# tobifinn/torch-assimilate

Hardware: AMD Instinct MI355X
Metric: local analyses/sec (LETKF, 40-member) (higher is better)
Workload: dtype f32

## Files before the change

### include/mia_letkf.h

```cpp
#ifndef MIA_LETKF_H
#define MIA_LETKF_H

#include <stddef.h>
#include <stdint.h>

#ifdef __cplusplus
extern "C" {
#endif

#define MIA_VERSION 100

#define MIA_OK 0
#define MIA_ERR_NULL (-1)
#define MIA_ERR_SIZE (-2)
#define MIA_ERR_UNSUPPORTED (-3)
#define MIA_ERR_WORKSPACE (-4)
#define MIA_ERR_ALIGN (-5)
#define MIA_ERR_COMM (-6)
#define MIA_ERR_ARG (-7)

#define MIA_FLAG_OVERFLOW 1
#define MIA_FLAG_NOCONV 2
#define MIA_FLAG_NONFINITE 4
#define MIA_FLAG_RETRY 8
#define MIA_FLAG_MASK 0xff

#define MIA_TAPER_GC 0
#define MIA_TAPER_GC_INF 1

#define MIA_MAX_COORD 3
#define MIA_MAX_RADII 3

int mia_version(void);
const char* mia_status_string(int status);

int mia_set_option(const char* name, int value);
int mia_get_option(const char* name, int* value);
int mia_last_analysis_kernel(char* buf, int n);
int mia_last_transform_kernel(char* buf, int n);

int mia_gaspari_cohn_f64(const double* r, int64_t n, double* w, void* stream);
int mia_gaspari_cohn_f32(const float* r, int64_t n, float* w, void* stream);
int mia_gaspari_cohn_inf_f64(const double* r, int64_t n, double* w, void* stream);
int mia_gaspari_cohn_inf_f32(const float* r, int64_t n, float* w, void* stream);

int mia_letkf_localize_workspace_bytes(int64_t P, int n_coord, size_t* bytes);
int mia_letkf_localize_f64(const double* grid_xyz, int64_t g0, int64_t g1,
                           const double* obs_xyz, int64_t P, int n_coord,
                           const int32_t* coord_group ,
                           const double* gc_c , int n_r, double gc_eps,
                           int p_cap, int32_t* nbr_cnt, int32_t* nbr_idx, double* nbr_w,
                           int32_t* stats, void* ws, size_t ws_bytes, void* stream);

int mia_letkf_localize_taper_f64(int taper, const double* grid_xyz, int64_t g0, int64_t g1,
                                 const double* obs_xyz, int64_t P, int n_coord,
                                 const int32_t* coord_group , const double* gc_c , int n_r,
                                 double gc_eps, int p_cap, int32_t* nbr_cnt, int32_t* nbr_idx, double* nbr_w,
                                 int32_t* stats, void* ws, size_t ws_bytes, void* stream);

int mia_letkf_index_build_f64(const double* obs_xyz, int64_t P, int n_coord,
                              const int32_t* coord_group , const double* gc_c , int n_r,
                              void* ws, size_t ws_bytes , void* stream);

int mia_letkf_localize_taper_periodic_f64(int taper, const double* grid_xyz, int64_t g0, int64_t g1,
                                          const double* obs_xyz, int64_t P, int n_coord,
                                          const int32_t* coord_group , const double* period ,
                                          const double* gc_c , int n_r, double gc_eps, int p_cap, int32_t* nbr_cnt, int32_t* nbr_idx, double* nbr_w,
                                          int32_t* stats, void* ws, size_t ws_bytes, void* stream);
int mia_letkf_index_build_periodic_f64(const double* obs_xyz, int64_t P, int n_coord,
                                       const int32_t* coord_group , const double* period ,
                                       const double* gc_c , int n_r, void* ws, size_t ws_bytes, void* stream);

// ... 427 lines not shown
```

### torch-assimilate_amd/_build.py

```python
import hashlib
import os
import shutil
import subprocess

HERE = os.path.dirname(os.path.abspath(__file__))
ROOT = os.path.dirname(HERE)
CSRC = os.path.join(HERE, "csrc")
LIB_DIR = os.path.join(HERE, "lib")
LIB_PATH = os.path.join(LIB_DIR, "libmia_letkf.so")
STAMP = os.path.join(LIB_DIR, "libmia_letkf.stamp")
SOURCES = ["localize.hip", "letkf_entry.hip", "etkf_global.hip", "letkf_wave.hip", "letkf_sys.hip", "letkf_cheb.hip", "letkf_tile.hip", "letkf_tile_split.hip", "letkf_tile64.hip", "letkf_tile64w.hip", "letkf_dense64.hip", "letkf_patch64.hip", "letkf_stream64.hip", "letkf_stream64w.hip", "letkf_patch64w.hip", "letkf_wide64.hip", "letkf_wide64w.hip", "letkf_tile2.hip", "letkf_tile2w.hip", "letkf_tile2p.hip", "letkf_tile2f.hip", "lketkf_tile.hip", "lketkf_tile64.hip", "lketkf_kern64.hip", "tile_lists.hip", "sharded_step.hip", "step_comm.hip", "obs_space.hip", "ienks.hip", "lienks_tile64.hip", "lienks_wide64.hip", "lienks_stream64.hip", "apply_local.hip", "apply_local64.hip", "api.cc"]
HEADERS = ["mia_common.h", "mia_options.h", "mia_jacobi.h", "mia_jacobi_sym.h", "mia_kernel_prog.h", "mia_localize_dev.h", "mia_kernels.h", "mia_cheb_table64.h", "mia_pack_dev.h", "mia_step_comm.h", "mia_tiles.h", "mia_tile_launch.h", "mia_frames64.h", os.path.join(ROOT, "include", "mia_letkf.h")]
INCLUDES = {"letkf_tile_split.hip": ["letkf_tile.hip"], "lketkf_kern64.hip": ["lketkf_tile64.hip"]}
SOURCE_FLAGS = {"letkf_tile2.hip": ["-fno-slp-vectorize"], "letkf_tile2w.hip": ["-fno-slp-vectorize"], "letkf_tile2p.hip": ["-fno-slp-vectorize"],
                "letkf_tile2f.hip": ["-fno-slp-vectorize"]}
FLAGS = ["--offload-arch=gfx950", "-O3", "-std=c++17", "-fPIC", "-shared",
         "-I" + os.path.join(ROOT, "include"), "-I" + CSRC]


def _flags():
    return FLAGS + os.environ.get("MIA_BUILD_FLAGS", "").split()


def _sources():
    return [os.path.join(CSRC, s) for s in SOURCES if os.path.exists(os.path.join(CSRC, s))]


def _digest():
    h = hashlib.sha256()
    for f in _sources() + [f if os.path.isabs(f) else os.path.join(CSRC, f) for f in HEADERS]:
        with open(f, "rb") as fh:
            h.update(fh.read())
    h.update(" ".join(_flags()).encode())
    return h.hexdigest()


def hipcc_path():
    return shutil.which("hipcc") or "/opt/rocm/bin/hipcc"


def _object_digest(src):
    h = hashlib.sha256()
    for f in [src] + [f if os.path.isabs(f) else os.path.join(CSRC, f) for f in HEADERS + INCLUDES.get(os.path.basename(src), [])]:
        with open(f, "rb") as fh:
            h.update(fh.read())
# ... 54 lines not shown
```

### torch-assimilate_amd/_cabi.py

```python
import ctypes as C
import os

from ._build import LIB_PATH

_lib = None

i32, i64, f32, f64, vp, sz = C.c_int, C.c_int64, C.c_float, C.c_double, C.c_void_p, C.c_size_t


class KernelOp(C.Structure):
    _fields_ = [("op", C.c_int32), ("reserved", C.c_int32), ("value", C.c_double)]


_LISTS = [vp, vp, vp, i32, i32]
_SHARD = [vp, i64, i32, i32, i64, i64, vp, i64] + _LISTS


def _analysis_entry(f):
    return (_SHARD + [f, f, vp, i64, i64, vp, vp, vp], i32)


def _analysis_redo(f):
    return (_SHARD + [f, f, vp, i64, i64, vp, vp], i32)


def _weights_entry(f):
    return (_SHARD + [f, f, vp, i64, i64, vp, vp, vp, vp], i32)


def _ienks_tile_entry(f):
    return ([vp, i64, i32, i64, i64, vp, i64] + _LISTS + [f, vp, vp, vp, vp], i32)


_COVER7 = ([i32, i32, i32, i64, i64, i64, i64], i32)
_COVER4 = ([i32, i32, i64, i64], i32)

_PROTOS = {
    "mia_version": ([], i32),
    "mia_status_string": ([i32], C.c_char_p),
    "mia_set_option": ([C.c_char_p, i32], i32),
    "mia_get_option": ([C.c_char_p, C.POINTER(C.c_int)], i32),
    "mia_last_analysis_kernel": ([C.c_char_p, i32], i32),
    "mia_last_transform_kernel": ([C.c_char_p, i32], i32),
    "mia_gaspari_cohn_f64": ([vp, i64, vp, vp], i32),
    "mia_gaspari_cohn_f32": ([vp, i64, vp, vp], i32),
    "mia_gaspari_cohn_inf_f64": ([vp, i64, vp, vp], i32),
    "mia_gaspari_cohn_inf_f32": ([vp, i64, vp, vp], i32),
    "mia_letkf_localize_taper_f64": ([i32, vp, i64, i64, vp, i64, i32, C.POINTER(C.c_int32), C.POINTER(f64), i32, f64,
                                      i32, vp, vp, vp, vp, vp, sz, vp], i32),
    "mia_letkf_localize_from_dist_taper_f64": ([i32, vp, vp, i64, i32, C.POINTER(f64), i32, f64, vp, vp, vp, vp, vp],
                                               i32),
    "mia_lketkf_kernel_analysis_packed_f32": ([vp, i64, i32, i32, i64, i64, vp, i64, vp, vp, vp, i32, i32, f32,
                                               C.POINTER(KernelOp), i32, vp, i64, i64, vp, vp, vp], i32),
    "mia_lketkf_kernel_analysis_packed_f64": ([vp, i64, i32, i32, i64, i64, vp, i64, vp, vp, vp, i32, i32, f64,
                                               C.POINTER(KernelOp), i32, vp, i64, i64, vp, vp, vp], i32),
    "mia_letkf_localize_workspace_bytes": ([i64, i32, C.POINTER(sz)], i32),
    "mia_letkf_localize_f64": ([vp, i64, i64, vp, i64, i32, C.POINTER(C.c_int32), C.POINTER(f64), i32, f64,
                                i32, vp, vp, vp, vp, vp, sz, vp], i32),
    "mia_letkf_localize_from_dist_f64": ([vp, vp, i64, i32, C.POINTER(f64), i32, f64, vp, vp, vp, vp, vp], i32),
    "mia_letkf_analysis_workspace_bytes": ([i32, i64, i32, C.POINTER(sz)], i32),
    "mia_letkf_analysis_f32": ([vp, i64, i32, i32, i64, i64, vp, vp, i64, vp, vp, vp, i32, i32, f32,
                                vp, i64, i64, vp, vp, vp, sz, vp], i32),
    "mia_letkf_analysis_f64": ([vp, i64, i32, i32, i64, i64, vp, vp, i64, vp, vp, vp, i32, i32, f64,
                                vp, i64, i64, vp, vp, vp, sz, vp], i32),
    "mia_letkf_pack_obs_f32": ([vp, vp, i32, i64, vp, vp], i32),
    "mia_letkf_pack_obs_f64": ([vp, vp, i32, i64, vp, vp], i32),
    "mia_letkf_analysis_packed_f32": _analysis_entry(f32),
    "mia_letkf_analysis_packed_f64": _analysis_entry(f64),
    "mia_letkf_analysis_matfun_f32": _analysis_entry(f32),
    "mia_letkf_analysis_matfun_f64": _analysis_entry(f64),
    "mia_letkf_analysis_retry_f64": _analysis_redo(f64),
    "mia_letkf_matfun_f64_cover": _COVER7,
    "mia_letkf_analysis_dense_f64": _analysis_entry(f64),
    "mia_letkf_dense_f64_cover": _COVER7,
    "mia_letkf_analysis_patch_f64": ([vp, i64, i32, i32, i64, i64, vp, i64, vp, vp, vp, i32, i32, f64, f64,
                                      vp, i64, i64, vp, vp, vp, i64, i32, vp], i32),
# ... 221 lines not shown
```

### torch-assimilate_amd/csrc/api.cc

```cpp
#include "mia_letkf.h"

extern "C" int mia_version(void) { return MIA_VERSION; }

extern "C" const char* mia_status_string(int status) {
  switch (status) {
    case MIA_OK: return "ok";
    case MIA_ERR_NULL: return "required pointer is NULL";
    case MIA_ERR_SIZE: return "invalid or inconsistent size argument";
    case MIA_ERR_UNSUPPORTED: return "shape not supported by the gfx950 kernels (LDS capacity / index range)";
    case MIA_ERR_WORKSPACE: return "workspace too small (use the *_workspace_bytes query)";
    case MIA_ERR_ALIGN: return "workspace pointer must be 256-byte aligned";
    case MIA_ERR_COMM: return "RCCL / communicator failure (mia_comm_last_error has the detail)";
    case MIA_ERR_ARG: return "invalid argument value (e.g. a negative or non-finite period)";
    default: return status > 0 ? "HIP runtime error (value is the hipError_t)" : "unknown status";
  }
}

#include <atomic>
#include <cstring>
#include "mia_options.h"

namespace mia {
static std::atomic<int> g_opt[MIA_OPT_COUNT_] = {62, 1, 1, 1, 1, 1, 1, 1, 1, 1, 1, 1, 1, 1};
static thread_local const int* t_override = nullptr;
int option(int id) {
  if (id < 0 || id >= MIA_OPT_COUNT_) return 0;
  return t_override ? t_override[id] : g_opt[id].load(std::memory_order_relaxed);
}
void option_snapshot(int* out) { for (int i = 0; i < MIA_OPT_COUNT_; ++i) out[i] = g_opt[i].load(std::memory_order_relaxed); }
void option_override(const int* snapshot) { t_override = snapshot; }
static std::atomic<int> g_apply64{-1};
int option_apply64() { return g_apply64.load(std::memory_order_relaxed); }
}

#include <cstdarg>
#include <cstdio>
#include <mutex>
namespace mia {
static std::mutex g_last_mu;
static char g_last_kernel[160] = "";
void note_analysis_kernel(const char* fmt, ...) {
  char buf[sizeof(g_last_kernel)];
  va_list ap;
  va_start(ap, fmt);
  vsnprintf(buf, sizeof(buf), fmt, ap);
  va_end(ap);
  std::lock_guard<std::mutex> lk(g_last_mu);
  memcpy(g_last_kernel, buf, sizeof(buf));
}
}

extern "C" int mia_last_analysis_kernel(char* buf, int n) {
  if (!buf || n < 1) return MIA_ERR_NULL;
  std::lock_guard<std::mutex> lk(mia::g_last_mu);
  snprintf(buf, (size_t)n, "%s", mia::g_last_kernel);
  return MIA_OK;
}

namespace mia {
static char g_last_transform[160] = "";
void note_transform_kernel(const char* fmt, ...) {
  char buf[sizeof(g_last_transform)];
  va_list ap;
  va_start(ap, fmt);
  vsnprintf(buf, sizeof(buf), fmt, ap);
  va_end(ap);
// ... 39 lines not shown
```

### torch-assimilate_amd/csrc/letkf_tile2.hip

```cpp
#include "mia_common.h"
#include <hip/hip_ext.h>
#include "mia_kernels.h"
#include "mia_options.h"
#include "mia_tiles.h"
#include "mia_tile_launch.h"
#include "letkf_tile2_kernel.h"

namespace mia {


template <int UT, int KT, bool MROWS, int WAVES>
__global__ __launch_bounds__(64, WAVES)
void letkf_tile2_kernel(Tile2Params P) { tile2_body<UT, KT, MROWS, 0>(P, nullptr, (int64_t)blockIdx.y * gridDim.x + blockIdx.x); }

#ifdef MIA_TILE_STAMPS
extern "C" int mia_debug_tile2_stamps(long long* host, int n_tiles) {
  if (n_tiles > kT2StampTiles) n_tiles = kT2StampTiles;
  return (int)hipMemcpyFromSymbol(host, HIP_SYMBOL(g_tile2_stamps), sizeof(long long) * kT2StampN * (size_t)n_tiles);
}
#endif

size_t tile2_lds_bytes(int ut, int k) {
  return (size_t)ut * split_nc8(k) * 512 + 512 + (size_t)16 * ut * 12;
}

template <int UT, int KT, bool MROWS>
constexpr int tile2_waves() { return UT <= 2 && KT <= 4 ? (MROWS ? 2 : MIA_TILE2_WAVES_UT2) : (UT <= 3 && KT <= 4 && !MROWS ? 2 : 1); }

template <int UT, int KT, bool MROWS, int WAVES = tile2_waves<UT, KT, MROWS>()>
static int tile2_launch_m(const Tile2Params& tp, hipStream_t stream) {
  size_t lds = tile2_lds_bytes(UT, tp.k);
  {
    int per_cu = 0;
    MIA_EXP_SET(per_cu, "MIA_TILE2_WAVES_PER_CU", atoi);
    if (per_cu > 0 && (size_t)(160 * 1024) / per_cu > lds) lds = ((size_t)(160 * 1024) / per_cu) & ~(size_t)255;
  }
  return launch_blocks_carried(letkf_tile2_kernel<UT, KT, MROWS, WAVES>, (tp.ng + 15) >> 4, 64, lds, stream, [] {
    note_analysis_kernel("letkf_tile2_kernel<%d, %d, %s, %d>", UT, KT, MROWS ? "true" : "false", WAVES);
  }, tp);
}

template <int UT, int KT>
static int tile2_launch_s(const Tile2Params& tp, hipStream_t stream) {
#ifdef MIA_EXPERIMENTS
  if constexpr (UT == 2 && KT == 3) {
    int w = 0;
    MIA_EXP_SET(w, "MIA_TILE2_WAVES", atoi);
    if (tp.m == 1 && w == 5) return tile2_launch_m<UT, KT, false, 5>(tp, stream);
    if (tp.m == 1 && w == 6) return tile2_launch_m<UT, KT, false, 6>(tp, stream);
    if (tp.m == 1 && w == 3) return tile2_launch_m<UT, KT, false, 3>(tp, stream);
  }
#endif
  bool force_rows = false;
  MIA_EXP_SET(force_rows, "MIA_TILE2_FORCE_MROWS", (bool)atoi);
  return tp.m == 1 && !force_rows ? tile2_launch_m<UT, KT, false>(tp, stream) : tile2_launch_m<UT, KT, true>(tp, stream);
}

template <int UT>
static int tile2_launch_u(const Tile2Params& tp, int kt, hipStream_t stream) {
  return dispatch_upto<6>(kt, [&](auto kt_c) {
    if constexpr (kt_c() >= 5 || UT <= kt_c() + 1) return tile2_launch_s<UT, kt_c()>(tp, stream);
    else return MIA_ERR_UNSUPPORTED;
  });
}

bool tile2_covers(int m, int k, int p_max, int extra_blocks, int64_t ldx, int64_t ldo, int64_t ng) {
  if (!(m >= 1 && k >= 2 && k <= 96 && p_max <= k && extra_blocks >= 0)) return false;
  if ((int64_t)k * ldx * 4 >= ((int64_t)1 << 31) || (int64_t)k * ldo * 4 >= ((int64_t)1 << 31)) return false;
  const int kt = (k + 15) >> 4, ut = tile_ut_for(p_max) + extra_blocks;
  if (ut > kt + 1 || ut > 6) return false;
  if (tile2_lds_bytes(ut, k) > kMaxDynamicLds) return false;
  return grid_covers((ng + 15) >> 4);
}

bool tile2_records_addressable(int k, int64_t P) { return (P + 1) * (int64_t)split_rec_bytes(k) < ((int64_t)1 << 32); }

int tile2_analysis_launch(const float* X, int64_t ldx, int m, int k, int64_t g0, int64_t ng, const void* rec, int64_t P,
                          const void* tile_lists, int ut, float inf_factor, float* Xa, int64_t ldo, int64_t o0,
                          int32_t* flags, int32_t* retry_count, int dmax, const int2* tab_hdr, const float2* tab_c,
                          hipStream_t stream, int seg_len, int64_t seg_stride, const Tile2Housekeeping* hk, const Tile2Loc* loc) {
  if (seg_len < 0 || (seg_len & 15) || (seg_len > 0 && ng >= ((int64_t)1 << 31))) return MIA_ERR_UNSUPPORTED;
  if (!flags || !retry_count || !tab_hdr || !tab_c || !tile_lists || !rec) return MIA_ERR_UNSUPPORTED;
  const int kt = (k + 15) >> 4;
  if (ut < 1 || ut > 6 || ut > kt + 1 || !tile2_covers(m, k, 0, ut - 1, ldx, ldo, ng)) return MIA_ERR_UNSUPPORTED;
  if (!tile2_records_addressable(k, P)) return MIA_ERR_UNSUPPORTED;
  const TileListLayout L = tile_list_layout(ng, ut);
  const char* base = (const char*)tile_lists;
  Tile2Params tp;
  tp.X = X; tp.ldx = ldx; tp.m = m; tp.k = k; tp.g0 = g0; tp.ng = ng;
  tp.rec = (const unsigned char*)rec; tp.rb = split_rec_bytes(k); tp.nc8 = split_nc8(k); tp.zero_rec = P;
  tp.thdr = (const int4*)(base + L.hdr); tp.tidx = (const int32_t*)(base + L.idx); tp.tD = (const f4w*)(base + L.D);
  const double rg = (double)(k - 1) / (double)inf_factor, km = (double)(k - 1);
  tp.inv_reg = (float)(1.0 / rg);
  tp.f0 = (float)sqrt(km / rg);
  tp.inv_k = (float)(1.0 / (double)k);
  tp.cs_phi = (float)(sqrt(km) / (rg * sqrt(rg)));
  tp.cs_psi = (float)(1.0 / rg);
  tp.Xa = Xa; tp.ldo = ldo; tp.o0 = o0; tp.flags = flags; tp.retry_count = retry_count; tp.dmax = dmax;
  tp.tab_hdr = tab_hdr; tp.tab_c = tab_c;
  tp.seg_len = seg_len; tp.seg_stride = seg_stride;
  tp.clr_counts = hk ? hk->counts : nullptr; tp.clr_n = hk ? hk->n : nullptr; tp.clr_err = hk ? hk->err : nullptr;
  tp.err_out = hk ? hk->err_out : nullptr;
  tp.stagger = 0;
  MIA_EXP_SET(tp.stagger, "MIA_TILE2_STAGGER", atoi);
  { int pm = 0, tr = 0; MIA_EXP_SET(pm, "MIA_TILE2_PRIO", atoi); MIA_EXP_SET(tr, "MIA_TILE2_TRIM", atoi); tp.stagger |= (pm & 0xff) << 8 | tr << 16; }
  if (loc) return tile2f_launch(tp, *loc, ut, kt, stream);
  if (ut >= 3 && option(MIA_OPT_TILE_PAIR) != 0) {
    const int prc = tile2p_launch_any(tp, ut, kt, stream);
    if (prc != MIA_ERR_UNSUPPORTED) return prc;
  }
#ifdef MIA_TILE2_SINGLE
  if (ut == 2 && kt == 3) return tile2_launch_s<2, 3>(tp, stream);
  return MIA_ERR_UNSUPPORTED;
#else
  return dispatch_upto<6>(ut, [&](auto ut_c) { return tile2_launch_u<ut_c()>(tp, kt, stream); });
#endif
}

}

using namespace mia;

extern "C" int mia_letkf_analysis_tiles_f32(const float* X, int64_t ldx, int m, int k, int64_t g0, int64_t g1,
                                            const void* split_rec, int64_t P, const void* tile_lists, int p_max,
                                            int extra_blocks, float inf_factor, float* Xa, int64_t ldo, int64_t o0, int32_t* flags,
                                            int32_t* retry_count, void* stream_) {
  (void)hipGetLastError();
  hipStream_t stream = (hipStream_t)stream_;
  if (m < 1 || k < 2 || g1 < g0 || g0 < 0 || P < 0 || p_max < 0 || extra_blocks < 0 || !(inf_factor > 0.0f)) return MIA_ERR_SIZE;
  if (g1 == g0) return MIA_OK;
  if (!X || !Xa || !split_rec || !tile_lists || !flags || !retry_count) return MIA_ERR_NULL;
  if (!tile2_covers(m, k, p_max, extra_blocks, ldx, ldo, g1 - g0)) return MIA_ERR_UNSUPPORTED;
  const int2* th = nullptr;
  const float2* tc = nullptr;
  if (!cheb_dual_table(stream, &th, &tc)) return MIA_ERR_UNSUPPORTED;
  return tile2_analysis_launch(X, ldx, m, k, g0, g1 - g0, split_rec, P, tile_lists, tile_ut_for(p_max) + extra_blocks, inf_factor, Xa,
// ... 3 lines not shown
```

### torch-assimilate_amd/csrc/letkf_tile2_kernel.h

```cpp
#pragma once
#include <type_traits>
#include "mia_common.h"
#include <hip/hip_ext.h>
#include "mia_kernels.h"
#include "mia_options.h"
#include "mia_tiles.h"
#ifdef MIA_TILE_STAMPS
namespace mia { constexpr int kT2StampN = 20, kT2StampTiles = 8192; static __device__ long long g_tile2_stamps[kT2StampTiles * kT2StampN]; }
#define MIA_TL_STAMP(i) do { if (lane == 0 && tile < mia::kT2StampTiles) mia::g_tile2_stamps[tile * mia::kT2StampN + 12 + (i)] = (long long)__builtin_amdgcn_s_memtime(); } while (0)
#endif
#include "mia_tile_localize.h"

namespace mia {

#ifdef MIA_TILE_STAMPS
#define T2_STAMP(i) do { if (lane == 0 && bid < kT2StampTiles) g_tile2_stamps[bid * kT2StampN + (i)] = (long long)__builtin_amdgcn_s_memtime(); } while (0)
#define T2_STAMP_HWID() do { if (lane == 0 && bid < kT2StampTiles) g_tile2_stamps[bid * kT2StampN + 9] = \
    (long long)(unsigned)__builtin_amdgcn_s_getreg((31 << 11) | 4) | ((long long)(unsigned)__builtin_amdgcn_s_getreg((31 << 11) | 20) << 32); } while (0)
#define T2_STAMP_REAL(i) do { if (lane == 0 && bid < kT2StampTiles) g_tile2_stamps[bid * kT2StampN + (i)] = (long long)__builtin_amdgcn_s_memrealtime(); } while (0)
#else
#define T2_STAMP(i) do { } while (0)
#define T2_STAMP_HWID() do { } while (0)
#define T2_STAMP_REAL(i) do { } while (0)
#endif

#ifndef MIA_TILE2_WAVES_UT2
#define MIA_TILE2_WAVES_UT2 4
#endif

template <int UT, int KT, bool MROWS, int LOC>
__device__ __forceinline__ void tile2_body(Tile2Params P, const Tile2Loc* loc, const int64_t bid) {
  constexpr int UMAX = 16 * UT, NB = (KT + 1) / 2, NKB = (UT + 1) / 2;
  extern __shared__ __attribute__((aligned(16))) unsigned char smem[];
  int lane = threadIdx.x, lr = lane & 15, h = lane >> 4;
  const int k = P.k, nc8 = P.nc8;
  const unsigned IMG = (unsigned)(UT * nc8) * 512u;
  unsigned char* zline = smem + IMG;
  int* ukey = reinterpret_cast<int*>(smem + IMG + 512);
  float* wdl = reinterpret_cast<float*>(ukey + UMAX);
  float* El = wdl + UMAX;

  const int64_t ntile = (P.ng + 15) >> 4;
  if (bid >= ntile) return;
  if (P.clr_counts) {
    const int ncl = *P.clr_n;
    for (int64_t i = bid * 64 + lane; i < ncl; i += ntile * 64) P.clr_counts[i] = 0;
    if (bid == 0 && lane == 0) {
      const unsigned e = *P.clr_err;
      if (e) { atomicOr(P.err_out, (int)(e << 3)); *P.clr_err = 0u; }
    }
  }
  const int64_t q8 = ntile >> 3, r8 = ntile & 7, xcd = bid & 7;
  const int64_t tile = (xcd < r8 ? xcd * (q8 + 1) : r8 * (q8 + 1) + (xcd - r8) * q8) + (bid >> 3);
  const int64_t p0 = tile << 4;
  const int npts = P.ng - p0 < 16 ? (int)(P.ng - p0) : 16;
  int64_t oc0 = P.o0 + p0;
  if (P.seg_len > 0) {
    const unsigned sgi = (unsigned)p0 / (unsigned)P.seg_len;
    oc0 = p0 - (int64_t)sgi * P.seg_len;
    P.Xa += (int64_t)sgi * P.seg_stride;
  }
  const unsigned ldxb = (unsigned)P.ldx * 4u, ldob = (unsigned)P.ldo * 4u;
  int lrc = lr < npts ? lr : npts - 1;
  bool colok = lr < npts;

#ifdef MIA_EXPERIMENTS
  const int prio_mode = (P.stagger >> 8) & 0xff, exp_trim = P.stagger >> 16;
  P.stagger &= 0xff;
  if (prio_mode == 1) __builtin_amdgcn_s_setprio(3);
  if (prio_mode >= 3) {
    const int wid = (int)(__builtin_amdgcn_s_getreg((4 << 11) | 4) & 0xf);
    const bool fast = prio_mode == 3 ? (wid & 1) : (prio_mode == 4 ? wid < 2 : (prio_mode == 5 ? wid == 0 : (wid % 3) == 0));
    if (fast) __builtin_amdgcn_s_setprio(3);
  }
  if (P.stagger > 0) {
    const int slot = (int)(__builtin_amdgcn_s_getreg((4 << 11) | 4) & 0xf);
    for (int i = 0; i < slot * P.stagger; ++i) __builtin_amdgcn_s_sleep(1);
  }
#endif
  T2_STAMP(0);
  T2_STAMP_HWID();
  T2_STAMP_REAL(10);
  int hdU = 0;
  int myidx[(UMAX + 63) / 64];
  f4w dreg[UT];
  if constexpr (LOC == 0) {
// ... 455 lines not shown
```

### torch-assimilate_amd/csrc/letkf_tile2f.hip

```cpp
#include "mia_common.h"
#include <hip/hip_ext.h>
#include "mia_kernels.h"
#include "mia_options.h"
#include "mia_tiles.h"
#include "mia_tile_launch.h"
#include "letkf_tile2_kernel.h"

namespace mia {

struct Tile2FParams { Tile2Params t; Tile2Loc loc; };

template <int UT, int KT, int NC, bool MROWS, int WAVES>
__global__ __launch_bounds__(64, WAVES)
void letkf_tile2f_kernel(Tile2FParams PF) { tile2_body<UT, KT, MROWS, NC>(PF.t, &PF.loc, (int64_t)blockIdx.y * gridDim.x + blockIdx.x); }

#ifdef MIA_TILE_STAMPS
extern "C" int mia_debug_tile2f_stamps(long long* host, int n_tiles) {
  if (n_tiles > kT2StampTiles) n_tiles = kT2StampTiles;
  return (int)hipMemcpyFromSymbol(host, HIP_SYMBOL(g_tile2_stamps), sizeof(long long) * kT2StampN * (size_t)n_tiles);
}
#endif

bool tile2f_covers(int m, int k, int ut, int n_coord) {
  const int kt = (k + 15) >> 4;
  return m >= 1 && ut >= 1 && ut <= 2 && kt >= 1 && kt <= 6 && n_coord >= 1 && n_coord <= MIA_MAX_COORD;
}

template <int UT, int KT, int NC, bool MROWS>
static int tile2f_launch_m(const Tile2FParams& pf, hipStream_t stream) {
  const size_t a = tile2_lds_bytes(UT, pf.t.k), b = tile_loc_lds(UT);
  const size_t lds = a > b ? a : b;
  constexpr int WAVES = MROWS ? 2 : MIA_TILE2_WAVES_UT2;
  return launch_blocks_carried(letkf_tile2f_kernel<UT, KT, NC, MROWS, WAVES>, (pf.t.ng + 15) >> 4, 64, lds, stream, [] {
    note_analysis_kernel("letkf_tile2f_kernel<%d, %d, %d, %s, %d>", UT, KT, NC, MROWS ? "true" : "false", WAVES);
  }, pf);
}

template <int UT, int KT, int NC>
static int tile2f_launch_n(const Tile2FParams& pf, hipStream_t stream) {
  return pf.t.m == 1 ? tile2f_launch_m<UT, KT, NC, false>(pf, stream) : tile2f_launch_m<UT, KT, NC, true>(pf, stream);
}

template <int UT>
static int tile2f_launch_u(const Tile2FParams& pf, int kt, hipStream_t stream) {
  return dispatch_upto<6>(kt, [&](auto kt_c) {
    return dispatch_among<7, 6, 5, 3, 2, 1>(pf.loc.scan.nc + (pf.loc.periodic ? 4 : 0), [&](auto nc) { return tile2f_launch_n<UT, kt_c(), nc()>(pf, stream); });
  });
}

int tile2f_launch(const Tile2Params& tp, const Tile2Loc& loc, int ut, int kt, hipStream_t stream) {
  if (!tile2f_covers(tp.m, tp.k, ut, loc.scan.nc) || !loc.stats) return MIA_ERR_UNSUPPORTED;
  Tile2FParams pf;
  pf.t = tp;
  pf.loc = loc;
#ifdef MIA_TILE2_SINGLE
  if (ut == 2 && kt == 3 && loc.scan.nc == 1) return tile2f_launch_n<2, 3, 1>(pf, stream);
  return MIA_ERR_UNSUPPORTED;
#else
  return ut == 1 ? tile2f_launch_u<1>(pf, kt, stream) : tile2f_launch_u<2>(pf, kt, stream);
#endif
}

}
```

### torch-assimilate_amd/csrc/mia_tile_launch.h

```cpp
#pragma once
#include <hip/hip_ext.h>
#include <type_traits>
#include <utility>
#include "mia_common.h"
#include "mia_kernels.h"

namespace mia {

constexpr int64_t kGridColumns = 65536, kGridMaxRows = 65535;
constexpr int64_t kGridMaxBlocks = kGridColumns * kGridMaxRows;
static inline bool grid_covers(int64_t n) { return n <= kGridMaxBlocks; }
static inline bool launch_grid(int64_t n, dim3* grid) {
  const int64_t gx = n < kGridColumns ? n : kGridColumns;
  const int64_t gy = (n + gx - 1) / gx;
  if (gy > kGridMaxRows) return false;
  *grid = dim3((unsigned)gx, (unsigned)gy);
  return true;
}

template <bool CARRIED, typename Note, typename... KArgs, typename... Args>
static inline int launch_blocks_impl(void (*kern)(KArgs...), int64_t n_blocks, unsigned block, size_t lds, hipStream_t stream, Note&& note,
                                     const Args&... args) {
  if (lds > kMaxDynamicLds) return MIA_ERR_UNSUPPORTED;
  if (lds > 48 * 1024) MIA_HIP_TRY(hipFuncSetAttribute((const void*)kern, hipFuncAttributeMaxDynamicSharedMemorySize, (int)lds));
  dim3 grid;
  if (!launch_grid(n_blocks, &grid)) return MIA_ERR_UNSUPPORTED;
  if constexpr (CARRIED) {
    hipEvent_t& stop = launch_stop_event();
    if (stop) {
      hipExtLaunchKernelGGL(kern, grid, dim3(block), (unsigned)lds, stream, launch_start_event(), stop, 0, args...);
      stop = nullptr;
      launch_start_event() = nullptr;
    } else {
      kern<<<grid, dim3(block), lds, stream>>>(args...);
    }
    ++tile_launch_count();
  } else {
    kern<<<grid, dim3(block), lds, stream>>>(args...);
  }
  note();
  MIA_LAUNCH_CHECK();
  return MIA_OK;
}
template <typename Note, typename... KArgs, typename... Args>
static inline int launch_blocks(void (*kern)(KArgs...), int64_t n_blocks, unsigned block, size_t lds, hipStream_t stream, Note&& note,
                                const Args&... args) {
  return launch_blocks_impl<false>(kern, n_blocks, block, lds, stream, note, args...);
}
template <typename Note, typename... KArgs, typename... Args>
static inline int launch_blocks_carried(void (*kern)(KArgs...), int64_t n_blocks, unsigned block, size_t lds, hipStream_t stream, Note&& note,
                                        const Args&... args) {
  return launch_blocks_impl<true>(kern, n_blocks, block, lds, stream, note, args...);
}
static inline void no_note() {}

template <int... Vs, typename F>
static inline int dispatch_among(int v, F&& f) {
  int rc = MIA_ERR_UNSUPPORTED;
  (void)((v == Vs ? (rc = f(std::integral_constant<int, Vs>{}), true) : false) || ...);
  return rc;
}
template <typename F, int... Is>
static inline int dispatch_upto_impl(int v, F&& f, std::integer_sequence<int, Is...>) { return dispatch_among<(int)(sizeof...(Is) - Is)...>(v, f); }
template <int N, typename F>
static inline int dispatch_upto(int v, F&& f) { return dispatch_upto_impl(v, f, std::make_integer_sequence<int, N>{}); }

}
```

### torch-assimilate_amd/csrc/mia_tiles.h

```cpp
#pragma once
#include "mia_common.h"

namespace mia {

constexpr int kTileSlack = 8;

static inline int tile_ut_for(int p_max) {
  const int ut = (p_max + kTileSlack + 15) >> 4;
  return ut < 1 ? 1 : ut;
}

struct TileListLayout { size_t hdr, idx, D, bytes; int ut; int64_t ntile; };
static inline TileListLayout tile_list_layout(int64_t ng, int ut) {
  TileListLayout L;
  L.ut = ut;
  L.ntile = (ng + 15) >> 4;
  size_t o = 0;
  L.hdr = o; o = align_up(o + (size_t)(L.ntile > 0 ? L.ntile : 1) * 16, 256);
  L.idx = o; o = align_up(o + (size_t)(L.ntile > 0 ? L.ntile : 1) * 16 * ut * sizeof(int32_t), 256);
  L.D = o; o = align_up(o + (size_t)(L.ntile > 0 ? L.ntile : 1) * ut * 1024, 256);
  L.bytes = o;
  return L;
}

// ... 285 lines not shown
  unsigned char* o = J.rec + j * rb;
  const float E = bad ? __builtin_nanf("") : __uint_as_float((unsigned)(127 - es) << 23);
  *reinterpret_cast<f4w*>(o + 32 * nc8) = f4w{wd, E, 0.0f, 0.0f};
  for (int c = 0; c < nc8; ++c) {
    float x[8];
#pragma unroll
    for (int i = 0; i < 8; ++i) x[i] = (real && 8 * c + i < k) ? lds[(8 * c + i) * 64 + lane] * sc : 0.0f;
    h8v hi, lo;
    split8(x, hi, lo);
    *reinterpret_cast<h8v*>(o + 32 * c) = hi;
    *reinterpret_cast<h8v*>(o + 32 * c + 16) = lo;
  }
}
static inline size_t split_pack_lean_lds(int k) { return (size_t)64 * k * sizeof(float); }

struct ScanParams;
int split_pack_launch(const float* Yb, const float* d, int k, int64_t P, void* rec, hipStream_t stream);
int tile_lists_launch(const double* grid_xyz, int64_t g0, int64_t ng, int64_t P, int n_coord, const int32_t* coord_group,
                      const double* gc_c, int n_r, double gc_eps, int taper, int ut, void* tile_lists, int32_t* stats,
                      void* index_ws, hipStream_t stream, const SplitPackJob* pack, bool bucket = false, const int* counts = nullptr,
                      const double* period = nullptr);
struct Tile2Params {
  const float* X; int64_t ldx; int m, k;
  int64_t g0, ng;
  const unsigned char* rec; int rb, nc8; int64_t zero_rec;
  const int4* thdr; const int32_t* tidx; const f4w* tD;
  float inv_reg, f0, inv_k, cs_phi, cs_psi;
  float* Xa; int64_t ldo, o0; int32_t* flags; int32_t* retry_count;
  int dmax;
  const int2* tab_hdr; const float2* tab_c;
  int seg_len; int64_t seg_stride;
  int* clr_counts; const int* clr_n; unsigned* clr_err; int32_t* err_out;
  int stagger;
};
struct Tile2Housekeeping { int* counts; const int* n; unsigned* err; int32_t* err_out; };
bool tile2_covers(int m, int k, int p_max, int extra_blocks, int64_t ldx, int64_t ldo, int64_t ng);
bool tile2_records_addressable(int k, int64_t P);
int tile2_analysis_launch(const float* X, int64_t ldx, int m, int k, int64_t g0, int64_t ng, const void* rec, int64_t P,
                          const void* tile_lists, int ut, float inf_factor, float* Xa, int64_t ldo, int64_t o0,
                          int32_t* flags, int32_t* retry_count, int dmax, const int2* tab_hdr, const float2* tab_c,
                          hipStream_t stream, int seg_len = 0, int64_t seg_stride = 0, const Tile2Housekeeping* hk = nullptr,
                          const struct Tile2Loc* loc = nullptr);
bool tile2f_covers(int m, int k, int ut, int n_coord);
int tile2f_launch(const Tile2Params& tp, const struct Tile2Loc& loc, int ut, int kt, hipStream_t stream);
size_t tile2_lds_bytes(int ut, int k);

int tile2p_launch_any(const Tile2Params& tp, int ut, int kt, hipStream_t stream);
bool lketkf_tile_covers(int m, int k, int p_max, int extra_blocks, int64_t ldx, int64_t ldo, int64_t ng, int64_t P);
int lketkf_tile_launch(const float* X, int64_t ldx, int m, int k, int64_t g0, int64_t ng, const float* Yb, const float* d,
                       int64_t P, const void* tile_lists, int ut, float inf_factor, float gamma, float* Xa, int64_t ldo,
                       int64_t o0, int32_t* flags, int32_t* retry_count, int dmax, const int2* tab_hdr, const float2* tab_c,
                       hipStream_t stream, int seg_len = 0, int64_t seg_stride = 0, const Tile2Housekeeping* hk = nullptr);

}
```

### torch-assimilate_amd/engine.py

```python
from __future__ import annotations

import ctypes as C
import warnings
from dataclasses import dataclass
from typing import Optional, Sequence

import torch

from . import _cabi

__all__ = ["LetkfEngine", "NeighbourLists", "ObsIndex", "mesh_tiles"]


def _ptr(t: Optional[torch.Tensor]):
    return None if t is None else C.c_void_p(t.data_ptr())


def _one_of(names) -> str:
    return ", ".join(repr(v) for v in names[:-1]) + " or " + repr(names[-1])


def _result(out, W, flags, finish, defer_retry):
    if not defer_retry:
        if finish is not None:
# ... 99 lines not shown

@dataclass
class ObsIndex:
    ws: torch.Tensor
    obs: torch.Tensor
    radii: list
    coord_group: list
    P: int
    nc: int
    period: Optional[list] = None


def _periods(period, nc: int):
    if period is None:
        return None
    per = [0.0 if p is None else float(p) for p in (period if hasattr(period, "__len__") else [period] * nc)]
    if len(per) != nc:
        raise ValueError("period needs one entry per coordinate")
    if any(not (p >= 0.0 and p < float("inf")) for p in per):
        raise ValueError("period must be finite and >= 0")
    if not any(p > 0.0 for p in per):
        return None
    return (C.c_double * nc)(*per)


def _period_arg(per, nc: int):
    return per if per is not None else (C.c_double * nc)()


class LetkfEngine:

    def __init__(self, device: Optional[torch.device] = None):
        self.lib = _cabi.lib()
        if not torch.cuda.is_available():
            raise _cabi.MiaError("no MI355X visible: the LETKF hot path has no CPU fallback")
        self.device = torch.device(device if device is not None else "cuda:%d" % torch.cuda.current_device())
        self._ws = {}
        self._p_cap_hint = 32

    def _stream(self):
        return C.c_void_p(torch.cuda.current_stream(self.device).cuda_stream)

    def _workspace(self, tag: str, nbytes: int) -> torch.Tensor:
        cur = self._ws.get(tag)
        if cur is None or cur.numel() < nbytes:
            cur = torch.empty(max(int(nbytes), 256), dtype=torch.uint8, device=self.device)
            assert cur.data_ptr() % 256 == 0
            self._ws[tag] = cur
        return cur

    def _dev(self, a, dtype):
        t = torch.as_tensor(a)
        return t.to(device=self.device, dtype=dtype).contiguous()

    def _redo_behind_counter(self, retry: torch.Tensor, entry: str, redo_args, alive=()):
        def finish(_alive=alive):
            n_retry = int(retry.item())
            if n_retry:
                _cabi.check(getattr(self.lib, entry)(*redo_args(), self._stream()), entry)
            return n_retry
        return finish

    def gaspari_cohn(self, r: torch.Tensor, taper: int = 0) -> torch.Tensor:
        r = r.to(self.device).contiguous()
        out = torch.empty_like(r)
        name = "mia_gaspari_cohn_" + ("inf_" if taper else "") + {torch.float64: "f64", torch.float32: "f32"}[r.dtype]
# ... 909 lines not shown
```

### torch-assimilate_amd/sharded.py

```python
from __future__ import annotations

from typing import Callable, List, Optional, Sequence, Tuple

import os
import torch

__all__ = ["ShardedLetkf", "PendingStep", "block_partition", "gather_blocks"]


TILE_BOX_OVERFLOW = 1 << 30
STATUS_NONFINITE = 128
STATUS_SAMPLED = 64


def block_partition(G: int, world: int) -> List[Tuple[int, int]]:
    n = (G + world - 1) // world
    return [(min(G, r * n), min(G, (r + 1) * n)) for r in range(world)]


def gather_blocks(shard: torch.Tensor, G: int, world: int, group=None) -> torch.Tensor:
    import torch.distributed as dist
    if world == 1:
        return shard
    m, k, n_r = shard.shape
# ... 137 lines not shown
        import ctypes as C
        from .engine import _ptr
        lib, comm = self.engine.lib, st["comm"]
        parts = block_partition(G, self.world)
        g0, g1 = parts[self.rank]
        col = torch.arange(G, device=self.device, dtype=torch.float32)
        ctr = torch.zeros(8, dtype=torch.int32, device=self.device)
        ok = True
        for s, buf in enumerate(bufs):
            flat = buf.view(rows, G)
            flat.fill_(-1.0)
            pat = lambda r, a, b: (r + 1) * 4096.0 + (col[a:b] % 61.0)[None] + (torch.arange(rows, device=self.device) % 64)[:, None] * 64.0
            flat[:, g0:g1] = pat(self.rank, g0, g1)
            torch.cuda.synchronize(self.device)
            ctr.zero_()
            ctr[0] = 100 + self.rank
            rc = lib.mia_comm_peer_exchange(comm, s, rows, G, g0, g1, _ptr(ctr), C.c_void_p(torch.cuda.current_stream(self.device).cuda_stream))
            torch.cuda.synchronize(self.device)
            want = torch.empty_like(flat)
            for r, (a, b) in enumerate(parts):
                want[:, a:b] = pat(r, a, b)
            c = ctr.tolist()
            ok = ok and rc == 0 and bool(torch.equal(flat, want)) and c[4] == 100 + self.world - 1 and c[7] == 0
        return ok

    def __init__(self, device, rank: int = 0, world: int = 1, radii: Sequence[float] = (10.0,),
                 inf_factor: float = 1.0, coord_group: Optional[Sequence[int]] = None, eps: float = 1e-5,
                 rbf_gamma: Optional[float] = None, compute_shard: Optional[Callable] = None, group=None,
                 method: str = "auto", fused_localization: bool = False,
                 comm_chunks: int = 4, chunk_compute: Optional[Callable] = None, native_step: bool = True,
                 max_in_flight: int = 3, peer_exchange: str = "auto", copy_results: bool = True, prep_streams: int = 3,
                 analysis_streams: int = 3, gather: bool = True, fuse_tile_lists="auto", prep_priority: int = 0, period=None):
        self.device, self.rank, self.world = device, rank, world
        self.radii, self.inf_factor, self.coord_group, self.eps = list(radii), inf_factor, coord_group, eps
        self.period = period
        self.rbf_gamma = rbf_gamma
        self.gather = bool(gather)
        self.method = method
        self.fused_localization = fused_localization
        self.fuse_tile_lists = fuse_tile_lists
        self.comm_chunks = int(comm_chunks)
        self._chunk_compute = chunk_compute
        self._comm_stream = None
        self._obuf = None
        self.native_step = native_step
        self._native = None
        self._in_flight = []
        self._time_next = False
        self.kernel_timings = []
        self.max_in_flight = max(1, min(int(max_in_flight), 16))
        self.prep_streams = max(0, min(int(prep_streams), 8))
        self.analysis_streams = max(1, min(int(analysis_streams), 4))
        self.prep_priority = int(prep_priority)
        self.peer_rewaits = 3
        self._peer_rewait_hook = None
        self.peer_exchange = peer_exchange
        self.copy_results = copy_results
        self._submitted = 0
        self.reused_steps = 0
        self._force_comm = False
        self.native_steps = 0
        self.last_retries = 0
        self.group = group
        self._engine = None
        self._compute = compute_shard or self._engine_shard
        self.last_p_max = 0
# ... 907 lines not shown
```

Before: 2.612 billion.

## Pack multiple tile wavefronts per workgroup in tile2 LETKF kernels

Tile2 kernels previously launched one 64-thread wavefront per block. Each workgroup now holds up to four wavefronts (default 4, set by MIA_TILE_WPG), each processing its own tile in a private LDS slice. The XCD-aware tile mapping now applies at group granularity. This cuts the block count and may improve scheduling and occupancy, but it raises launch bounds to 256 threads, which can constrain registers, and it couples four waves' LDS into one allocation.

```diff
diff --git a/include/mia_letkf.h b/include/mia_letkf.h
--- a/include/mia_letkf.h
+++ b/include/mia_letkf.h
@@ -38,6 +38,8 @@
 int mia_get_option(const char* name, int* value);
 int mia_last_analysis_kernel(char* buf, int n);
 int mia_last_transform_kernel(char* buf, int n);
+int mia_tile_wpg_from_env(void);
+int mia_tile_wpg(void);
 
 int mia_gaspari_cohn_f64(const double* r, int64_t n, double* w, void* stream);
 int mia_gaspari_cohn_f32(const float* r, int64_t n, float* w, void* stream);
diff --git a/torch-assimilate_amd/_build.py b/torch-assimilate_amd/_build.py
--- a/torch-assimilate_amd/_build.py
+++ b/torch-assimilate_amd/_build.py
@@ -10,7 +10,7 @@
 LIB_PATH = os.path.join(LIB_DIR, "libmia_letkf.so")
 STAMP = os.path.join(LIB_DIR, "libmia_letkf.stamp")
 SOURCES = ["localize.hip", "letkf_entry.hip", "etkf_global.hip", "letkf_wave.hip", "letkf_sys.hip", "letkf_cheb.hip", "letkf_tile.hip", "letkf_tile_split.hip", "letkf_tile64.hip", "letkf_tile64w.hip", "letkf_dense64.hip", "letkf_patch64.hip", "letkf_stream64.hip", "letkf_stream64w.hip", "letkf_patch64w.hip", "letkf_wide64.hip", "letkf_wide64w.hip", "letkf_tile2.hip", "letkf_tile2w.hip", "letkf_tile2p.hip", "letkf_tile2f.hip", "lketkf_tile.hip", "lketkf_tile64.hip", "lketkf_kern64.hip", "tile_lists.hip", "sharded_step.hip", "step_comm.hip", "obs_space.hip", "ienks.hip", "lienks_tile64.hip", "lienks_wide64.hip", "lienks_stream64.hip", "apply_local.hip", "apply_local64.hip", "api.cc"]
-HEADERS = ["mia_common.h", "mia_options.h", "mia_jacobi.h", "mia_jacobi_sym.h", "mia_kernel_prog.h", "mia_localize_dev.h", "mia_kernels.h", "mia_cheb_table64.h", "mia_pack_dev.h", "mia_step_comm.h", "mia_tiles.h", "mia_tile_launch.h", "mia_frames64.h", os.path.join(ROOT, "include", "mia_letkf.h")]
+HEADERS = ["mia_common.h", "mia_options.h", "mia_jacobi.h", "mia_jacobi_sym.h", "mia_kernel_prog.h", "mia_localize_dev.h", "mia_kernels.h", "mia_cheb_table64.h", "mia_pack_dev.h", "mia_step_comm.h", "mia_tiles.h", "mia_tile_launch.h", "mia_tile_map.h", "mia_tile_localize.h", "letkf_tile2_kernel.h", "mia_frames64.h", os.path.join(ROOT, "include", "mia_letkf.h")]
 INCLUDES = {"letkf_tile_split.hip": ["letkf_tile.hip"], "lketkf_kern64.hip": ["lketkf_tile64.hip"]}
 SOURCE_FLAGS = {"letkf_tile2.hip": ["-fno-slp-vectorize"], "letkf_tile2w.hip": ["-fno-slp-vectorize"], "letkf_tile2p.hip": ["-fno-slp-vectorize"],
                 "letkf_tile2f.hip": ["-fno-slp-vectorize"]}
diff --git a/torch-assimilate_amd/_cabi.py b/torch-assimilate_amd/_cabi.py
--- a/torch-assimilate_amd/_cabi.py
+++ b/torch-assimilate_amd/_cabi.py
@@ -42,6 +42,8 @@
     "mia_get_option": ([C.c_char_p, C.POINTER(C.c_int)], i32),
     "mia_last_analysis_kernel": ([C.c_char_p, i32], i32),
     "mia_last_transform_kernel": ([C.c_char_p, i32], i32),
+    "mia_tile_wpg_from_env": ([], i32),
+    "mia_tile_wpg": ([], i32),
     "mia_gaspari_cohn_f64": ([vp, i64, vp, vp], i32),
     "mia_gaspari_cohn_f32": ([vp, i64, vp, vp], i32),
     "mia_gaspari_cohn_inf_f64": ([vp, i64, vp, vp], i32),
diff --git a/torch-assimilate_amd/csrc/api.cc b/torch-assimilate_amd/csrc/api.cc
--- a/torch-assimilate_amd/csrc/api.cc
+++ b/torch-assimilate_amd/csrc/api.cc
@@ -32,6 +32,26 @@
 static std::atomic<int> g_apply64{-1};
 int option_apply64() { return g_apply64.load(std::memory_order_relaxed); }
 }
+
+#include <cstdlib>
+#include "mia_tile_map.h"
+namespace mia {
+static std::atomic<int> g_tile_wpg_log2{0};
+int tile_wpg_log2() { return g_tile_wpg_log2.load(std::memory_order_relaxed); }
+}
+
+extern "C" int mia_tile_wpg_from_env(void) {
+  const char* e = std::getenv("MIA_TILE_WPG");
+  int wpg = MIA_TILE_WPG;
+  if (e && *e) {
+    if (strcmp(e, "1") && strcmp(e, "2") && strcmp(e, "4")) return MIA_ERR_ARG;
+    wpg = e[0] - '0';
+  }
+  mia::g_tile_wpg_log2.store(mia::tile_wpg_log2_of(wpg), std::memory_order_relaxed);
+  return MIA_OK;
+}
+
+extern "C" int mia_tile_wpg(void) { return 1 << mia::tile_wpg_log2(); }
 
 #include <cstdarg>
 #include <cstdio>
diff --git a/torch-assimilate_amd/csrc/letkf_tile2.hip b/torch-assimilate_amd/csrc/letkf_tile2.hip
--- a/torch-assimilate_amd/csrc/letkf_tile2.hip
+++ b/torch-assimilate_amd/csrc/letkf_tile2.hip
@@ -10,7 +10,7 @@
 
 
 template <int UT, int KT, bool MROWS, int WAVES>
-__global__ __launch_bounds__(64, WAVES)
+__global__ __launch_bounds__(256, WAVES)
 void letkf_tile2_kernel(Tile2Params P) { tile2_body<UT, KT, MROWS, 0>(P, nullptr, (int64_t)blockIdx.y * gridDim.x + blockIdx.x); }
 
 #ifdef MIA_TILE_STAMPS
@@ -35,9 +35,10 @@
     MIA_EXP_SET(per_cu, "MIA_TILE2_WAVES_PER_CU", atoi);
     if (per_cu > 0 && (size_t)(160 * 1024) / per_cu > lds) lds = ((size_t)(160 * 1024) / per_cu) & ~(size_t)255;
   }
-  return launch_blocks_carried(letkf_tile2_kernel<UT, KT, MROWS, WAVES>, (tp.ng + 15) >> 4, 64, lds, stream, [] {
+  return tile_wave_launch(letkf_tile2_kernel<UT, KT, MROWS, WAVES>, tp, [](Tile2Params& p) -> Tile2Params& { return p; },
+                          (tp.ng + 15) >> 4, lds, stream, [] {
     note_analysis_kernel("letkf_tile2_kernel<%d, %d, %s, %d>", UT, KT, MROWS ? "true" : "false", WAVES);
-  }, tp);
+  });
 }
 
 template <int UT, int KT>
@@ -102,6 +103,7 @@
   tp.clr_counts = hk ? hk->counts : nullptr; tp.clr_n = hk ? hk->n : nullptr; tp.clr_err = hk ? hk->err : nullptr;
   tp.err_out = hk ? hk->err_out : nullptr;
   tp.stagger = 0;
+  tp.wave_shape = 0;
   MIA_EXP_SET(tp.stagger, "MIA_TILE2_STAGGER", atoi);
   { int pm = 0, tr = 0; MIA_EXP_SET(pm, "MIA_TILE2_PRIO", atoi); MIA_EXP_SET(tr, "MIA_TILE2_TRIM", atoi); tp.stagger |= (pm & 0xff) << 8 | tr << 16; }
   if (loc) return tile2f_launch(tp, *loc, ut, kt, stream);
diff --git a/torch-assimilate_amd/csrc/letkf_tile2_kernel.h b/torch-assimilate_amd/csrc/letkf_tile2_kernel.h
--- a/torch-assimilate_amd/csrc/letkf_tile2_kernel.h
+++ b/torch-assimilate_amd/csrc/letkf_tile2_kernel.h
@@ -5,6 +5,7 @@
 #include "mia_kernels.h"
 #include "mia_options.h"
 #include "mia_tiles.h"
+#include "mia_tile_map.h"
 #ifdef MIA_TILE_STAMPS
 namespace mia { constexpr int kT2StampN = 20, kT2StampTiles = 8192; static __device__ long long g_tile2_stamps[kT2StampTiles * kT2StampN]; }
 #define MIA_TL_STAMP(i) do { if (lane == 0 && tile < mia::kT2StampTiles) mia::g_tile2_stamps[tile * mia::kT2StampN + 12 + (i)] = (long long)__builtin_amdgcn_s_memtime(); } while (0)
@@ -14,10 +15,10 @@
 namespace mia {
 
 #ifdef MIA_TILE_STAMPS
-#define T2_STAMP(i) do { if (lane == 0 && bid < kT2StampTiles) g_tile2_stamps[bid * kT2StampN + (i)] = (long long)__builtin_amdgcn_s_memtime(); } while (0)
-#define T2_STAMP_HWID() do { if (lane == 0 && bid < kT2StampTiles) g_tile2_stamps[bid * kT2StampN + 9] = \
+#define T2_STAMP(i) do { if (lane == 0 && tile < kT2StampTiles) g_tile2_stamps[tile * kT2StampN + (i)] = (long long)__builtin_amdgcn_s_memtime(); } while (0)
+#define T2_STAMP_HWID() do { if (lane == 0 && tile < kT2StampTiles) g_tile2_stamps[tile * kT2StampN + 9] = \
     (long long)(unsigned)__builtin_amdgcn_s_getreg((31 << 11) | 4) | ((long long)(unsigned)__builtin_amdgcn_s_getreg((31 << 11) | 20) << 32); } while (0)
-#define T2_STAMP_REAL(i) do { if (lane == 0 && bid < kT2StampTiles) g_tile2_stamps[bid * kT2StampN + (i)] = (long long)__builtin_amdgcn_s_memrealtime(); } while (0)
+#define T2_STAMP_REAL(i) do { if (lane == 0 && tile < kT2StampTiles) g_tile2_stamps[tile * kT2StampN + (i)] = (long long)__builtin_amdgcn_s_memrealtime(); } while (0)
 #else
 #define T2_STAMP(i) do { } while (0)
 #define T2_STAMP_HWID() do { } while (0)
@@ -29,10 +30,12 @@
 #endif
 
 template <int UT, int KT, bool MROWS, int LOC>
-__device__ __forceinline__ void tile2_body(Tile2Params P, const Tile2Loc* loc, const int64_t bid) {
+__device__ __forceinline__ void tile2_body(Tile2Params P, const Tile2Loc* loc, const int64_t grp) {
   constexpr int UMAX = 16 * UT, NB = (KT + 1) / 2, NKB = (UT + 1) / 2;
-  extern __shared__ __attribute__((aligned(16))) unsigned char smem[];
-  int lane = threadIdx.x, lr = lane & 15, h = lane >> 4;
+  extern __shared__ __attribute__((aligned(16))) unsigned char smem_wg[];
+  const int wv = __builtin_amdgcn_readfirstlane((int)(threadIdx.x >> 6));
+  unsigned char* smem = smem_wg + (unsigned)wv * (P.wave_shape & ~3u);
+  int lane = threadIdx.x & 63, lr = lane & 15, h = lane >> 4;
   const int k = P.k, nc8 = P.nc8;
   const unsigned IMG = (unsigned)(UT * nc8) * 512u;
   unsigned char* zline = smem + IMG;
@@ -41,17 +44,16 @@
   float* El = wdl + UMAX;
 
   const int64_t ntile = (P.ng + 15) >> 4;
-  if (bid >= ntile) return;
+  const int64_t tile = tile_of_wave(grp, wv, ntile, (int)(P.wave_shape & 3u));
+  if (tile < 0) return;
   if (P.clr_counts) {
     const int ncl = *P.clr_n;
-    for (int64_t i = bid * 64 + lane; i < ncl; i += ntile * 64) P.clr_counts[i] = 0;
-    if (bid == 0 && lane == 0) {
+    for (int64_t i = tile * 64 + lane; i < ncl; i += ntile * 64) P.clr_counts[i] = 0;
+    if (tile == 0 && lane == 0) {
       const unsigned e = *P.clr_err;
       if (e) { atomicOr(P.err_out, (int)(e << 3)); *P.clr_err = 0u; }
     }
   }
-  const int64_t q8 = ntile >> 3, r8 = ntile & 7, xcd = bid & 7;
-  const int64_t tile = (xcd < r8 ? xcd * (q8 + 1) : r8 * (q8 + 1) + (xcd - r8) * q8) + (bid >> 3);
   const int64_t p0 = tile << 4;
   const int npts = P.ng - p0 < 16 ? (int)(P.ng - p0) : 16;
   int64_t oc0 = P.o0 + p0;
diff --git a/torch-assimilate_amd/csrc/letkf_tile2f.hip b/torch-assimilate_amd/csrc/letkf_tile2f.hip
--- a/torch-assimilate_amd/csrc/letkf_tile2f.hip
+++ b/torch-assimilate_amd/csrc/letkf_tile2f.hip
@@ -11,7 +11,7 @@
 struct Tile2FParams { Tile2Params t; Tile2Loc loc; };
 
 template <int UT, int KT, int NC, bool MROWS, int WAVES>
-__global__ __launch_bounds__(64, WAVES)
+__global__ __launch_bounds__(256, WAVES)
 void letkf_tile2f_kernel(Tile2FParams PF) { tile2_body<UT, KT, MROWS, NC>(PF.t, &PF.loc, (int64_t)blockIdx.y * gridDim.x + blockIdx.x); }
 
 #ifdef MIA_TILE_STAMPS
@@ -31,9 +31,10 @@
   const size_t a = tile2_lds_bytes(UT, pf.t.k), b = tile_loc_lds(UT);
   const size_t lds = a > b ? a : b;
   constexpr int WAVES = MROWS ? 2 : MIA_TILE2_WAVES_UT2;
-  return launch_blocks_carried(letkf_tile2f_kernel<UT, KT, NC, MROWS, WAVES>, (pf.t.ng + 15) >> 4, 64, lds, stream, [] {
+  return tile_wave_launch(letkf_tile2f_kernel<UT, KT, NC, MROWS, WAVES>, pf, [](Tile2FParams& p) -> Tile2Params& { return p.t; },
+                          (pf.t.ng + 15) >> 4, lds, stream, [] {
     note_analysis_kernel("letkf_tile2f_kernel<%d, %d, %d, %s, %d>", UT, KT, NC, MROWS ? "true" : "false", WAVES);
-  }, pf);
+  });
 }
 
 template <int UT, int KT, int NC>
diff --git a/torch-assimilate_amd/csrc/mia_tile_launch.h b/torch-assimilate_amd/csrc/mia_tile_launch.h
--- a/torch-assimilate_amd/csrc/mia_tile_launch.h
+++ b/torch-assimilate_amd/csrc/mia_tile_launch.h
@@ -4,8 +4,11 @@
 #include <utility>
 #include "mia_common.h"
 #include "mia_kernels.h"
+#include "mia_tile_map.h"
 
 namespace mia {
+
+int tile_wpg_log2();
 
 constexpr int64_t kGridColumns = 65536, kGridMaxRows = 65535;
 constexpr int64_t kGridMaxBlocks = kGridColumns * kGridMaxRows;
@@ -54,6 +57,25 @@
 }
 static inline void no_note() {}
 
+struct TileWaveShape { int wpg_log2; unsigned lds_slice, threads; int64_t blocks; size_t lds; };
+static inline TileWaveShape tile_wave_shape(int64_t ntile, size_t lds_wave, int wpg_log2) {
+  TileWaveShape s;
+  const size_t slice = align_up(lds_wave, kTileLdsSliceAlign);
+  while (wpg_log2 > 0 && (slice << wpg_log2) > kMaxDynamicLds) --wpg_log2;
+  s.wpg_log2 = wpg_log2;
+  s.lds_slice = (unsigned)slice;
+  s.threads = 64u << wpg_log2;
+  s.blocks = tile_groups(ntile, wpg_log2);
+  s.lds = wpg_log2 > 0 ? slice << wpg_log2 : lds_wave;
+  return s;
+}
+template <typename Note, typename KArg, typename Inner>
+static inline int tile_wave_launch(void (*kern)(KArg), KArg P, Inner&& p2, int64_t ntile, size_t lds_wave, hipStream_t stream, Note&& note) {
+  const TileWaveShape s = tile_wave_shape(ntile, lds_wave, tile_wpg_log2());
+  p2(P).wave_shape = s.lds_slice | (unsigned)s.wpg_log2;
+  return launch_blocks_carried(kern, s.blocks, s.threads, s.lds, stream, note, P);
+}
+
 template <int... Vs, typename F>
 static inline int dispatch_among(int v, F&& f) {
   int rc = MIA_ERR_UNSUPPORTED;
diff --git a/torch-assimilate_amd/csrc/mia_tile_map.h b/torch-assimilate_amd/csrc/mia_tile_map.h
--- /dev/null
+++ b/torch-assimilate_amd/csrc/mia_tile_map.h
@@ -0,0 +1,28 @@
+#pragma once
+
+#ifndef MIA_TILE_WPG
+#define MIA_TILE_WPG 4
+#endif
+static_assert(MIA_TILE_WPG == 1 || MIA_TILE_WPG == 2 || MIA_TILE_WPG == 4, "MIA_TILE_WPG: 1, 2 or 4 wavefronts per workgroup");
+
+namespace mia {
+
+constexpr unsigned kTileLdsSliceAlign = 512;
+
+constexpr int tile_wpg_log2_of(int wpg) { return wpg == 4 ? 2 : (wpg == 2 ? 1 : 0); }
+
+constexpr long long tile_groups(long long ntile, int wpg_log2) { return (ntile + (1ll << wpg_log2) - 1) >> wpg_log2; }
+
+constexpr long long xcd_item_of_block(long long b, long long n) {
+  const long long q8 = n >> 3, r8 = n & 7, xcd = b & 7;
+  return (xcd < r8 ? xcd * (q8 + 1) : r8 * (q8 + 1) + (xcd - r8) * q8) + (b >> 3);
+}
+
+constexpr long long tile_of_wave(long long g, int w, long long ntile, int wpg_log2) {
+  const long long ngroups = tile_groups(ntile, wpg_log2);
+  if (g >= ngroups) return -1;
+  const long long tile = (xcd_item_of_block(g, ngroups) << wpg_log2) + w;
+  return tile < ntile ? tile : -1;
+}
+
+}
diff --git a/torch-assimilate_amd/csrc/mia_tiles.h b/torch-assimilate_amd/csrc/mia_tiles.h
--- a/torch-assimilate_amd/csrc/mia_tiles.h
+++ b/torch-assimilate_amd/csrc/mia_tiles.h
@@ -341,6 +341,7 @@
   int seg_len; int64_t seg_stride;
   int* clr_counts; const int* clr_n; unsigned* clr_err; int32_t* err_out;
   int stagger;
+  unsigned wave_shape;
 };
 struct Tile2Housekeeping { int* counts; const int* n; unsigned* err; int32_t* err_out; };
 bool tile2_covers(int m, int k, int p_max, int extra_blocks, int64_t ldx, int64_t ldo, int64_t ng);
diff --git a/torch-assimilate_amd/engine.py b/torch-assimilate_amd/engine.py
--- a/torch-assimilate_amd/engine.py
+++ b/torch-assimilate_amd/engine.py
@@ -155,6 +155,7 @@
 
     def __init__(self, device: Optional[torch.device] = None):
         self.lib = _cabi.lib()
+        _cabi.check(self.lib.mia_tile_wpg_from_env(), "MIA_TILE_WPG")
         if not torch.cuda.is_available():
             raise _cabi.MiaError("no MI355X visible: the LETKF hot path has no CPU fallback")
         self.device = torch.device(device if device is not None else "cuda:%d" % torch.cuda.current_device())
diff --git a/torch-assimilate_amd/sharded.py b/torch-assimilate_amd/sharded.py
--- a/torch-assimilate_amd/sharded.py
+++ b/torch-assimilate_amd/sharded.py
@@ -193,6 +193,7 @@
                  max_in_flight: int = 3, peer_exchange: str = "auto", copy_results: bool = True, prep_streams: int = 3,
                  analysis_streams: int = 3, gather: bool = True, fuse_tile_lists="auto", prep_priority: int = 0, period=None):
         self.device, self.rank, self.world = device, rank, world
+        _cabi.check(_cabi.lib().mia_tile_wpg_from_env(), "MIA_TILE_WPG")
         self.radii, self.inf_factor, self.coord_group, self.eps = list(radii), inf_factor, coord_group, eps
         self.period = period
         self.rbf_gamma = rbf_gamma
```

New measurement: 2.640 billion, median of 2. About the same (+1.1%).
